# spaceandtimefdn/blitzar

Measured on NVIDIA H100. Metric: MSM throughput (scalar*point terms/sec), ristretto255, n=2^20 per GPU, higher is better.
Workload: dtype u32 limbs (integer modular arithmetic)

## Files before the change

### blitzar_b200/csrc/msm.cuh

```cuda
#pragma once
#include <algorithm>
#include <vector>

#include "batch_affine.cuh"
#include "curve.cuh"
#include "engine_api.cuh"
#include "lanefield.cuh"

namespace b200 {

struct ColumnDesc {
  const unsigned char* base;
  u64 row_stride;
  u32 bit_offset;
  u32 bit_width;
  u32 n;
  u32 is_signed;
  u32 first_window;
  u32 num_windows;
  u32 table_n;
  u32 gen_base;
};
B200_HD u32 bucket_windows(const ColumnDesc& col) { return col.table_n ? (col.num_windows ? 1u : 0u) : col.num_windows; }

B200_HD void load_scalar_bits(u32 v[8], bool& negative, const ColumnDesc& col, u64 i) {
  const unsigned char* row = col.base + i * col.row_stride;
#pragma unroll
  for (int k = 0; k < 8; ++k)
    v[k] = 0;
  const u32 width = col.bit_width;
  const unsigned char* p = row + (col.bit_offset >> 3);
  const u32 sh = col.bit_offset & 7u;
  if (sh == 0 && width == 256 && (((size_t)p) & 15u) == 0) {
    const uint4* q = (const uint4*)p;
    uint4 a = q[0], b = q[1];
    v[0] = a.x; v[1] = a.y; v[2] = a.z; v[3] = a.w;
    v[4] = b.x; v[5] = b.y; v[6] = b.z; v[7] = b.w;
  } else if (sh == 0 && (width & 31u) == 0 && (((size_t)p) & 3u) == 0) {
    const u32* q = (const u32*)p;
#pragma unroll
    for (int k = 0; k < 8; ++k)
      if ((u32)k < (width >> 5))
        v[k] = q[k];
  } else {
    const u32 nbytes = (sh + width + 7u) >> 3;
#pragma unroll
    for (int k = 0; k < 8; ++k) {
      u64 acc = 0;
#pragma unroll
      for (int b = 0; b < 5; ++b) {
        u32 idx = 4u * k + b;
        if (idx < nbytes)
          acc |= (u64)p[idx] << (8 * b);
      }
      v[k] = (u32)(acc >> sh);
    }
#pragma unroll
    for (int k = 0; k < 8; ++k) {
      int lo = 32 * k;
      if ((int)width <= lo)
        v[k] = 0;
      else if ((int)width < lo + 32)
        v[k] &= (1u << (width - lo)) - 1u;
    }
  }
  negative = false;
  if (col.is_signed) {
    u32 top = width - 1;
    bool neg = false;
#pragma unroll
    for (int k = 0; k < 8; ++k)
      if ((top >> 5) == (u32)k)
        neg = (v[k] >> (top & 31u)) & 1u;
    if (neg) {
      u64 c = 1;
#pragma unroll
      for (int k = 0; k < 8; ++k) {
        int lo = 32 * k;
        u32 m = 0;
        if ((int)width >= lo + 32)
          m = 0xffffffffu;
        else if ((int)width > lo)
          m = (1u << (width - lo)) - 1u;
        c += (u64)((~v[k]) & m);
        v[k] = (u32)c & m;
        c = (m == 0xffffffffu) ? (c >> 32) : 0;
      }
      negative = true;
    }
  }
}

constexpr u32 kAllWindows = 0xffffffffu;
template <class Fn>
B200_HD void for_each_digit(const u32 v[8], bool negative, const ColumnDesc& col, u32 c,
                            u32 nbuckets, Fn f, u32 only_window = kAllWindows) {
  const u32 half = nbuckets;
  const u32 mask = (1u << c) - 1u;
  u64 buf = 0;
  u32 nb = 0, w = 0, carry = 0;
  const u32 W = only_window == kAllWindows
                    ? col.num_windows
                    : (only_window < col.num_windows ? only_window + 1 : 0u);
  const auto step = [&] {
    u32 d = ((u32)buf & mask) + carry;
    buf >>= c;
    bool dneg = d > half;
    carry = dneg ? 1u : 0u;
    if (dneg)
      d = (1u << c) - d;
    if (d && (only_window == kAllWindows || w == only_window))
      f((col.first_window + (col.table_n ? 0u : w)) * nbuckets + (d - 1u), negative != dneg, w);
    ++w;
  };
#pragma unroll
  for (int k = 0; k < 8; ++k) {
    buf |= (u64)v[k] << nb;
    nb += 32;
    for (; nb >= c && w < W; nb -= c)
      step();
  }
  while (w < W)
    step();
}

B200_HD u32 column_of(const u64* col_start, u32 ncols, u64 tid) {
  u32 lo = 0, hi = ncols;
  while (hi - lo > 1) {
    const u32 mid = (lo + hi) >> 1;
    if (tid >= col_start[mid])
      lo = mid;
    else
      hi = mid;
  }
  return lo;
}
template <class Fn>
B200_HD void for_each_entry(const ColumnDesc* cols, const u64* col_start, u32 ncols, u32 c,
                            u32 nbuckets, u64 tid, Fn f, u32 only_window = kAllWindows) {
  const u32 j = column_of(col_start, ncols, tid);
  const ColumnDesc col = cols[j];
  if (only_window != kAllWindows && only_window >= col.num_windows)
    return;
  const u64 i = tid - col_start[j];
  u32 v[8];
  bool neg;
  load_scalar_bits(v, neg, col, i);
  const u32 ii = (u32)i + col.gen_base, tn = col.table_n;
  for_each_digit(v, neg, col, c, nbuckets, [&](u32 key, bool negate, u32 w) {
    f(key, make_entry(key, ii + w * tn, negate));
  }, only_window);
}

struct CountBody {
  static constexpr int kBlock = 256;
  const ColumnDesc* cols;
  const u64* col_start;
  u32 ncols, c, nbuckets;
  u32* counts;
  B200_HD void operator()(u64 tid) const {
    u32* cnt = counts;
    for_each_entry(cols, col_start, ncols, c, nbuckets, tid,
                   [cnt](u32 key, u64) { B200_ATOMIC_ADD(&cnt[key], 1u); });
  }
};

struct ScatterBody {
  static constexpr int kBlock = 256;
  const ColumnDesc* cols;
  const u64* col_start;
  u32 ncols, c, nbuckets;
  u32* cursor;
  u64* entries;
  u64 total_terms;
  B200_HD void operator()(u64 tid) const {
    u32 only = kAllWindows;
    if (total_terms) {
      only = (u32)(tid / total_terms);
      tid -= (u64)only * total_terms;
    }
    u32* cur = cursor;
    u64* en = entries;
    for_each_entry(cols, col_start, ncols, c, nbuckets, tid,
                   [cur, en](u32 key, u64 e) { en[B200_ATOMIC_ADD(&cur[key], 1u)] = e; }, only);
  }
};

constexpr u32 kScanChunk = 256, kScanChunkFirst = 64;
struct ScanUpBody {
  static constexpr int kBlock = 128;
  const u32* in;
  u64 n;
  u32* partial;
  u32 chunk;
  B200_HD void operator()(u64 t) const {
    u64 b = t * chunk, e = b + chunk < n ? b + chunk : n;
    u32 s = 0;
    for (u64 i = b; i < e; ++i)
      s += in[i];
    partial[t] = s;
  }
};
struct ScanTopBody {
  static constexpr int kBlock = 32;
  u32* data;
  u64 n;
  B200_HD void operator()(u64) const {
    u32 s = 0;
    for (u64 i = 0; i < n; ++i) {
      u32 v = data[i];
      data[i] = s;
      s += v;
    }
  }
};
struct ScanDownBody {
  static constexpr int kBlock = 128;
  u32* data;
  u64 n;
  const u32* partial_scanned;
  u32 chunk;
  B200_HD void operator()(u64 t) const {
    u64 b = t * chunk, e = b + chunk < n ? b + chunk : n;
    u32 s = partial_scanned[t];
    for (u64 i = b; i < e; ++i) {
      u32 v = data[i];
      data[i] = s;
      s += v;
    }
  }
};

inline void exclusive_scan(u32* data, u64 n, stream_t s, u32 chunk = kScanChunkFirst) {
  if (n <= kScanChunk) {
    launch(ScanTopBody{data, n}, 1, s);
    return;
  }
  u64 m = (n + chunk - 1) / chunk;
  u32* partial = (u32*)dev_alloc(m * sizeof(u32), s);
  launch(ScanUpBody{data, n, partial, chunk}, m, s);
  exclusive_scan(partial, m, s, kScanChunk);
  launch(ScanDownBody{data, n, partial, chunk}, m, s);
  dev_free(partial, s);
}

#if defined(__CUDACC__) && !defined(B200_EMULATE)
#define B200_BINNED_SORT 1
constexpr u32 kMicroBins = 16384, kBinCap = 8192, kBinSpan = 4096, kMaxBinShift = 12;
constexpr u64 kBinnedSortMinEntries = 1ull << 20;

template <int kBlock> __device__ u32 block_exclusive_scan(u32 v, u32* warp_sums, u32* total) {
  const u32 lane = threadIdx.x & 31u, warp = threadIdx.x >> 5;
  u32 x = v;
#pragma unroll
  for (int d = 1; d < 32; d <<= 1) {
    const u32 y = __shfl_up_sync(0xffffffffu, x, d);
    if (lane >= (u32)d)
      x += y;
  }
  if (lane == 31)
    warp_sums[warp] = x;
  __syncthreads();
  if (warp == 0) {
    u32 w = lane < kBlock / 32 ? warp_sums[lane] : 0u;
#pragma unroll
    for (int d = 1; d < 32; d <<= 1) {
      const u32 y = __shfl_up_sync(0xffffffffu, w, d);
      if (lane >= (u32)d)
        w += y;
    }
    if (lane < kBlock / 32)
      warp_sums[lane] = w;
  }
  __syncthreads();
  const u32 pre = (warp ? warp_sums[warp - 1] : 0u) + x - v;
  *total = warp_sums[kBlock / 32 - 1];
  __syncthreads();
  return pre;
}

struct MicroCountBody {
  static constexpr int kBlock = 512;
  const ColumnDesc* cols;
  const u64* col_start;
  u32 ncols, c, nbuckets;
  u64 total_terms;
  u32 tile, shift, nmicro;
  u32* micro_counts;
  __device__ void run(u32 b, unsigned char* smem) const {
    u32* h = (u32*)smem;
    for (u32 m = threadIdx.x; m < nmicro; m += kBlock)
      h[m] = 0;
    __syncthreads();
    const u64 lo = (u64)b * tile, hi = lo + tile < total_terms ? lo + tile : total_terms;
    const u32 sh = shift;
    for (u64 t = lo + threadIdx.x; t < hi; t += kBlock)
      for_each_entry(cols, col_start, ncols, c, nbuckets, t,
                     [h, sh](u32 key, u64) { atomicAdd(&h[key >> sh], 1u); });
    __syncthreads();
    for (u32 m = threadIdx.x; m < nmicro; m += kBlock)
      if (h[m])
        atomicAdd(&micro_counts[m], h[m]);
  }
};

struct PlanBinsBody {
  static constexpr int kBlock = 1024;
  const u32* micro_counts;
  u32 nmicro, span_micro;
  u64 nkeys;
  u32* bin_of;
  u32* bin_start;
  u32* bin_micro;
  u32* bin_cursor;
  u32* nbins_out;
  u32* counts;
  u32* d_m;
  __device__ bool starts_bin(const u32* st, u32 m) const {
    constexpr u32 H = kBinCap / 2;
    return m == 0 || m % span_micro == 0 || micro_counts[m] > H || micro_counts[m - 1] > H ||
           st[m] / H != st[m - 1] / H;
  }
  __device__ void run(u32, unsigned char* smem) const {
    __shared__ u32 ws[32];
    u32* st = (u32*)smem;
    const u32 per = (nmicro + kBlock - 1) / kBlock, m0 = min(threadIdx.x * per, nmicro),
              m1 = min(m0 + per, nmicro);
    u32 sum = 0;
    for (u32 m = m0; m < m1; ++m)
      sum += micro_counts[m];
    u32 total;
    u32 run = block_exclusive_scan<kBlock>(sum, ws, &total);
    for (u32 m = m0; m < m1; ++m) {
      st[m] = run;
      run += micro_counts[m];
    }
    __syncthreads();
    u32 nf = 0;
    for (u32 m = m0; m < m1; ++m)
      nf += starts_bin(st, m) ? 1u : 0u;
    u32 nbins;
    u32 id = block_exclusive_scan<kBlock>(nf, ws, &nbins);
    for (u32 m = m0; m < m1; ++m) {
      if (starts_bin(st, m)) {
        bin_start[id] = st[m];
        bin_micro[id] = m;
        bin_cursor[id] = st[m];
        ++id;
      }
      bin_of[m] = id - 1;
    }
    if (threadIdx.x == 0) {
      bin_start[nbins] = total;
      bin_micro[nbins] = nmicro;
      *nbins_out = nbins;
      counts[nkeys] = total;
      d_m[0] = total;
    }
  }
};

struct CoarseScatterBody {
  static constexpr int kBlock = 1024;
  const ColumnDesc* cols;
  const u64* col_start;
  u32 ncols, c, nbuckets;
  u64 total_terms;
  u32 tile, shift, nmicro;
  const u32* bin_of;
  const u32* nbins_ptr;
  u32* bin_cursor;
  u64* tmp;
  __device__ void run(u32 b, unsigned char* smem) const {
    __shared__ u32 ws[32];
    u32* h = (u32*)smem;
    u32* delta = h + nmicro;
    u64* stage = (u64*)(delta + nmicro + (nmicro & 1u));
    const u32 nbins = *nbins_ptr;
    for (u32 k = threadIdx.x; k < nbins; k += kBlock)
      h[k] = 0;
    __syncthreads();
    const u64 lo = (u64)b * tile, hi = lo + tile < total_terms ? lo + tile : total_terms;
    const u32 sh = shift;
    const u32* map = bin_of;
    for (u64 t = lo + threadIdx.x; t < hi; t += kBlock)
      for_each_entry(cols, col_start, ncols, c, nbuckets, t,
                     [h, sh, map](u32 key, u64) { atomicAdd(&h[__ldg(&map[key >> sh])], 1u); });
    __syncthreads();
    const u32 per = (nbins + kBlock - 1) / kBlock, k0 = min(threadIdx.x * per, nbins),
              k1 = min(k0 + per, nbins);
    u32 sum = 0;
    for (u32 k = k0; k < k1; ++k)
      sum += h[k];
    u32 size;
    u32 run = block_exclusive_scan<kBlock>(sum, ws, &size);
    for (u32 k = k0; k < k1; ++k) {
      const u32 n = h[k];
      if (n)
        delta[k] = atomicAdd(&bin_cursor[k], n) - run;
      h[k] = run;
      run += n;
    }
    __syncthreads();
    for (u64 t = lo + threadIdx.x; t < hi; t += kBlock)
      for_each_entry(cols, col_start, ncols, c, nbuckets, t, [h, sh, map, stage](u32 key, u64 e) {
        stage[atomicAdd(&h[__ldg(&map[key >> sh])], 1u)] = e;
      });
    __syncthreads();
    for (u32 i = threadIdx.x; i < size; i += kBlock) {
      const u64 e = stage[i];
      tmp[delta[__ldg(&map[entry_key(e) >> sh])] + i] = e;
    }
  }
};

struct BinSortBody {
  static constexpr int kBlock = 1024;
  static constexpr size_t kSmem = 2 * kBinCap * sizeof(u64) + kBinSpan * sizeof(u32);
  const u64* tmp;
  const u32* bin_start;
  const u32* bin_micro;
  const u32* nbins_ptr;
  u32 shift;
  u64 nkeys;
  u64* entries;
  u32* counts;
  __device__ void run(u32 b, unsigned char* smem) const {
    __shared__ u32 ws[32];
    if (b >= *nbins_ptr)
      return;
    u64* ent = (u64*)smem;
    u32* h = (u32*)(smem + 2 * kBinCap * sizeof(u64));
    const u32 lo = bin_start[b], size = bin_start[b + 1] - lo;
    const u64 klo = (u64)bin_micro[b] << shift, khi_m = (u64)bin_micro[b + 1] << shift;
    const u32 span = (u32)((khi_m < nkeys ? khi_m : nkeys) - klo);
    const bool local = size <= kBinCap;
    for (u32 k = threadIdx.x; k < span; k += kBlock)
      h[k] = 0;
    if (local) {
#pragma unroll 4
      for (u32 i = threadIdx.x; i < size; i += kBlock)
        ent[i] = tmp[(u64)lo + i];
    }
    __syncthreads();
    for (u32 i = threadIdx.x; i < size; i += kBlock) {
      const u64 e = local ? ent[i] : tmp[(u64)lo + i];
      atomicAdd(&h[entry_key(e) - (u32)klo], 1u);
    }
    __syncthreads();
    const u32 per = (span + kBlock - 1) / kBlock, k0 = min(threadIdx.x * per, span),
              k1 = min(k0 + per, span);
    u32 sum = 0;
    for (u32 k = k0; k < k1; ++k)
      sum += h[k];
    u32 total;
    u32 run = block_exclusive_scan<kBlock>(sum, ws, &total);
    for (u32 k = k0; k < k1; ++k) {
      const u32 n = h[k];
      h[k] = run;
      run += n;
      counts[klo + k] = lo + run;
    }
    __syncthreads();
    if (!local) {
      for (u32 i = threadIdx.x; i < size; i += kBlock) {
        const u64 e = tmp[(u64)lo + i];
        entries[(u64)lo + atomicAdd(&h[entry_key(e) - (u32)klo], 1u)] = e;
      }
      return;
    }
    u64* sorted = ent + kBinCap;
    for (u32 i = threadIdx.x; i < size; i += kBlock) {
      const u64 e = ent[i];
      sorted[atomicAdd(&h[entry_key(e) - (u32)klo], 1u)] = e;
    }
    __syncthreads();
    for (u32 i = threadIdx.x; i < size; i += kBlock)
      entries[(u64)lo + i] = sorted[i];
  }
};

inline u32 binned_sort_shift(u64 nkeys) {
  u32 shift = 0;
  while ((nkeys + (1ull << shift) - 1) >> shift > kMicroBins)
    ++shift;
  return shift;
}

inline void binned_sort(stream_t s, const ColumnDesc* d_cols, const u64* d_col_start, u32 ncols,
                        u32 c, u32 nbuckets, u64 total_terms, u64 max_entries, u32 max_windows,
                        u64 nkeys, u64* entries, u32* counts, u32* d_m) {
  const u32 shift = binned_sort_shift(nkeys);
  const u32 nmicro = (u32)((nkeys + (1ull << shift) - 1) >> shift);
  const u32 span_micro = std::max(1u, kBinSpan >> shift);
  u32* ws = (u32*)dev_alloc((5ull * nmicro + 3) * sizeof(u32), s);
  u32 *micro_counts = ws, *bin_of = ws + nmicro, *bin_cursor = ws + 2ull * nmicro,
      *bin_start = ws + 3ull * nmicro, *bin_micro = ws + 4ull * nmicro + 1,
      *nbins = ws + 5ull * nmicro + 2;
  u64* tmp = (u64*)dev_alloc(std::max<u64>(max_entries, 1) * sizeof(u64), s);
  dev_zero(micro_counts, nmicro * sizeof(u32), s);
  const u64 count_tile = 4096;
  launch_blocks(MicroCountBody{d_cols, d_col_start, ncols, c, nbuckets, total_terms,
                               (u32)count_tile, shift, nmicro, micro_counts},
                (total_terms + count_tile - 1) / count_tile, nmicro * sizeof(u32), s);
  launch_blocks(PlanBinsBody{micro_counts, nmicro, span_micro, nkeys, bin_of, bin_start, bin_micro,
                             bin_cursor, nbins, counts, d_m},
                1, nmicro * sizeof(u32), s);
  const size_t scatter_smem = 220 * 1024;
  const size_t bin_bytes = (2ull * nmicro + 2) * sizeof(u32);
  const u64 stage_entries = (scatter_smem - bin_bytes) / sizeof(u64);
  const u64 scatter_tile = std::max<u64>(1, stage_entries / max_windows);
  launch_blocks(CoarseScatterBody{d_cols, d_col_start, ncols, c, nbuckets, total_terms,
                                  (u32)scatter_tile, shift, nmicro, bin_of, nbins, bin_cursor, tmp},
                (total_terms + scatter_tile - 1) / scatter_tile, scatter_smem, s);
  launch_blocks(BinSortBody{tmp, bin_start, bin_micro, nbins, shift, nkeys, entries, counts}, nmicro,
                BinSortBody::kSmem, s);
  dev_free(tmp, s);
  dev_free(ws, s);
}
#endif

template <class C> struct FillIdentityBody {
  static constexpr int kBlock = 256;
  static constexpr u32 kChunks = sizeof(typename C::Point) / 16;
  static_assert(sizeof(typename C::Point) % 16 == 0, "points are made of 16-byte aligned fields");
  uint4* p;
  B200_HD void operator()(u64 t) const {
    const typename C::Point id = C::identity();
    const u32 k = (u32)(t % kChunks);
    uint4 v = ((const uint4*)&id)[0];
#pragma unroll
    for (u32 j = 1; j < kChunks; ++j)
      if (j == k)
        v = ((const uint4*)&id)[j];
    p[t] = v;
  }
};
template <class C> inline void fill_identity(stream_t s, typename C::Point* p, u64 n) {
  launch(FillIdentityBody<C>{(uint4*)p}, n * FillIdentityBody<C>::kChunks, s);
}

struct BucketOffsets {
  const u32* ends;
  const u32* starts;
  B200_HD u32 begin(u64 k) const { return starts ? starts[k] : (k ? ends[k - 1] : 0u); }
  B200_HD u32 end(u64 k) const { return ends[k]; }
};

template <class C> struct MergeBucketsBody {
  static constexpr int kBlock = 128;
  BucketOffsets offsets;
  const typename C::Point* scratch;
  typename C::Point* buckets;
  B200_HD void operator()(u64 k) const {
    if (offsets.begin(k) == offsets.end(k))
      return;
    typename C::Point b = buckets[k];
    C::add(b, b, scratch[k]);
    buckets[k] = b;
  }
};

template <class C, bool kGather, class X = SeqExec, bool kUniform = false, bool kUnitZ = false>
struct AccumulateBody {
  static constexpr int kBlock = 128;
  static constexpr int kMinBlocks = !kGather ? 1 : (C::F::N > 8 ? 2 : 3);
  typedef typename C::Point Point;
  typedef typename C::Gen Gen;
  const u32* keys;
  const u64* entries;
  const Gen* gens;
  const Point* pieces;
  const u32* m_ptr;
  u32 K;
  u32 final_level;
  Point* buckets;
  u32* out_keys;
  Point* out_pieces;
  u32* out_m_ptr;
  const u32* unit_veto;

  B200_HD void close_run(u64 t, u32 key, const Point& acc, bool writer, bool& first_seg) const {
    if (final_level || !first_seg) {
      if (writer)
        buckets[key] = acc;
    } else if (writer) {
      out_keys[2 * t] = key;
      out_pieces[2 * t] = acc;
    }
    first_seg = false;
  }
  template <bool kUnit> B200_HD Gen load_gen(u32 idx) const {
    if constexpr (kUnit)
      return C::load_unit_gen(gens + idx);
    else
      return gens[idx];
  }
  template <bool kUnit>
  B200_HD void gather_walk(u64 t, u64 b, u64 e, bool writer, u32& cur, Point& acc,
                           bool& first_seg) const {
    u64 ent = entries[b];
    Gen g = load_gen<kUnit>(entry_gen(ent));
    cur = entry_key(ent);
    for (u64 i = b; i < e; ++i) {
      u64 ent_n = ent;
      Gen g_n = g;
      if (i + 1 < e) {
        ent_n = entries[i + 1];
        g_n = load_gen<kUnit>(entry_gen(ent_n));
      }
      const u32 k = entry_key(ent);
      const bool negate = entry_negate(ent);
      if (kUniform) {
        if (i == b || k != cur) {
          if (i != b) {
            close_run(t, cur, acc, writer, first_seg);
            cur = k;
          }
          acc = C::identity();
        }
        C::template add_gen<X>(acc, acc, g, negate, kUnit);
      } else {
        const bool start = i == b || k != cur;
        if (k != cur) {
          close_run(t, cur, acc, writer, first_seg);
          cur = k;
        }
        if (start)
          C::gen_to_point(acc, g, negate);
        else
          C::template add_gen<X>(acc, acc, g, negate, kUnit);
      }
      ent = ent_n;
      g = g_n;
    }
  }
  B200_HD void operator()(u64 tid) const {
    const u64 t = tid / X::kLanes;
    const bool writer = (tid % X::kLanes) == 0;
    const u64 M = *m_ptr;
    const u64 T = (M + K - 1) / K;
    if (tid == 0 && out_m_ptr)
      *out_m_ptr = final_level ? 0u : (u32)(2 * T);
    u64 b = t * K;
    if (b >= M)
      return;
    u64 e = b + K < M ? b + K : M;
    u32 cur;
    Point acc;
    bool first_seg = true;
    if constexpr (kGather) {
      if (kUnitZ && unit_veto && *unit_veto)
        gather_walk<false>(t, b, e, writer, cur, acc, first_seg);
      else
        gather_walk<kUnitZ>(t, b, e, writer, cur, acc, first_seg);
    } else {
      cur = keys[b];
      acc = pieces[b];
      for (u64 i = b + 1; i < e; ++i) {
        const u32 k = keys[i];
        if (k == cur) {
          C::template add<X>(acc, acc, pieces[i]);
        } else {
          close_run(t, cur, acc, writer, first_seg);
          cur = k;
          acc = pieces[i];
        }
// ... 480 lines not shown
    if (kCommit)
      C::store_commit_abi(out + i * C::kAbiCommitBytes, pts[i]);
    else
      C::store_proj_abi(out + i * C::kAbiProjBytes, pts[i]);
  }
};
template <class C>
inline void launch_store_commit(stream_t s, const typename C::Point* pts, unsigned char* out,
                                u64 count, bool lane_tail) {
#ifdef B200_LANE_TAIL
  if constexpr (C::kCurveId == kRistretto255) {
    if (lane_tail && count && count <= 4096) {
      launch(StoreLaneBody{pts, out, count}, (count + 2) / 3 * 32, s);
      return;
    }
  }
#endif
  launch(StoreBody<C, true>{pts, out}, count, s);
}
template <class C> struct GenToProjBody {
  static constexpr int kBlock = 64;
  const typename C::Gen* gens;
  unsigned char* out;
  B200_HD void operator()(u64 i) const {
    typename C::Point p;
    C::gen_to_point(p, gens[i], false);
    C::store_proj_abi(out + i * C::kAbiProjBytes, p);
  }
};
template <class C> struct SumPartsBody {
  static constexpr int kBlock = 32;
  const typename C::Point* parts;
  u32 nparts, count;
  typename C::Point* out;
  B200_HD void operator()(u64 j) const {
    typename C::Point acc = parts[j];
    for (u32 r = 1; r < nparts; ++r)
      C::add(acc, acc, parts[(u64)r * count + j]);
    out[j] = acc;
  }
};

inline u32 choose_window_bits(u64 max_n, u32 max_width, u32 ncols, size_t point_bytes) {
  const double kMaxBucketBytes = 3.0e9;
  u32 best = 2;
  double best_cost = 1e300;
  for (u32 c = 2; c <= 16; ++c) {
    double W = (double)(max_width / c + 1);
    if (c > 8 && W * (double)(1u << (c - 1)) * (double)ncols * (double)point_bytes > kMaxBucketBytes)
      break;
    double cost = W * ((double)max_n + 2.5 * (double)(1u << (c - 1)));
    if (cost < best_cost) {
      best_cost = cost;
      best = c;
    }
  }
  return best;
}

struct MsmPlan {
  u32 c = 0, nbuckets = 0, ncols = 0, total_windows = 0;
  u64 nkeys = 0, max_n = 0, total_terms = 0, total_entries = 0;
  std::vector<ColumnDesc> cols;
};

inline MsmPlan msm_make_plan(std::vector<ColumnDesc> cols, const MsmOptions& opt,
                             size_t point_bytes) {
  MsmPlan p;
  p.ncols = (u32)cols.size();
  u32 max_width = 1;
  for (auto& col : cols) {
    p.max_n = std::max<u64>(p.max_n, col.n);
    p.total_terms += col.n;
    if (col.n)
      max_width = std::max(max_width, col.bit_width);
  }
  p.c = opt.window_bits ? opt.window_bits
                        : choose_window_bits(p.max_n, max_width, p.ncols, point_bytes);
  p.nbuckets = 1u << (p.c - 1);
  u64 max_entries = 0;
  for (auto& col : cols) {
    col.first_window = p.total_windows;
    col.num_windows = col.n ? col.bit_width / p.c + 1 : 0;
    p.total_windows += bucket_windows(col);
    max_entries += (u64)col.n * col.num_windows;
    if (col.table_n)
      B200_REQUIRE((u64)col.table_n * col.num_windows < (1ull << 31), "generator table too large");
    if (col.n)
      B200_REQUIRE((u64)col.gen_base + col.n + (u64)(col.num_windows - 1) * col.table_n < (1ull << 31),
                   "generator index of a column too large");
  }
  p.nkeys = (u64)p.total_windows * p.nbuckets;
  p.total_entries = max_entries;
  B200_REQUIRE(p.nkeys < (1ull << 32), "too many buckets for one pass");
  p.cols = std::move(cols);
  return p;
}

struct StagedRange {
  const ColumnDesc* d_cols = nullptr;
  const u64* d_col_start = nullptr;
  u64 total_terms = 0, max_entries = 0;
  u32 max_windows = 0;
  StagedRange(stream_t s, const MsmPlan& plan, u64 begin, u64 end) {
    const u32 ncols = plan.ncols;
    std::vector<ColumnDesc> cols(plan.cols);
    std::vector<u64> col_start(ncols + 1, 0);
    for (u32 j = 0; j < ncols; ++j) {
      u64 lo = std::min<u64>(begin, cols[j].n), hi = std::min<u64>(end, cols[j].n);
      cols[j].base += lo * cols[j].row_stride;
      cols[j].n = (u32)(hi - lo);
      col_start[j + 1] = col_start[j] + cols[j].n;
      max_entries += (u64)cols[j].n * cols[j].num_windows;
      max_windows = std::max(max_windows, cols[j].n ? cols[j].num_windows : 0u);
    }
    total_terms = col_start[ncols];
    if (total_terms == 0)
      return;
    B200_REQUIRE(max_entries < (1ull << 32) && end - begin < (1ull << 31),
                 "too many (term, window) entries for one sort pass");
    const size_t desc_bytes = ncols * sizeof(ColumnDesc), start_bytes = (ncols + 1) * sizeof(u64);
    std::vector<unsigned char> stage(desc_bytes + start_bytes);
    std::memcpy(stage.data(), cols.data(), desc_bytes);
    std::memcpy(stage.data() + desc_bytes, col_start.data(), start_bytes);
    d_cols = (const ColumnDesc*)stage_to_device(s, stage.data(), stage.size());
    d_col_start = (const u64*)((const unsigned char*)d_cols + desc_bytes);
  }
};

struct SortedLayout {
  u64* entries;
  u32* counts;
  u32* starts;
  u32* d_m;
  u64 slots_max;
  bool binned;
  BucketOffsets offsets() const { return {counts, starts}; }
};

inline SortedLayout sort_entries(stream_t s, const MsmPlan& plan, const StagedRange& r, u32 L,
                                 const MsmOptions& opt, u32* window_used) {
  const u32 ncols = plan.ncols, c = plan.c, nbuckets = plan.nbuckets;
  const u64 nkeys = plan.nkeys, max_entries = r.max_entries, total_terms = r.total_terms;
  SortedLayout out{};
  out.slots_max = L ? ((max_entries + nkeys * ((1ull << L) - 1) + (1ull << L) - 1) >> L) << L : max_entries;
  out.counts = (u32*)dev_alloc((nkeys + 1) * sizeof(u32), s);
  out.d_m = (u32*)dev_alloc(16 * sizeof(u32), s);
  out.entries = (u64*)dev_alloc(out.slots_max * sizeof(u64), s);
#ifdef B200_BINNED_SORT
  out.binned = L == 0 && opt.sort_path != 0 && binned_sort_shift(nkeys) <= kMaxBinShift &&
               (opt.sort_path == 2 || max_entries >= kBinnedSortMinEntries);
  if (out.binned)
    binned_sort(s, r.d_cols, r.d_col_start, ncols, c, nbuckets, total_terms, max_entries,
                r.max_windows, nkeys, out.entries, out.counts, out.d_m);
#endif
  if (!out.binned) {
    dev_zero(out.counts, (nkeys + 1) * sizeof(u32), s);
    launch(CountBody{r.d_cols, r.d_col_start, ncols, c, nbuckets, out.counts}, total_terms, s);
    if (L)
      launch(PadCountsBody{out.counts, (1u << L) - 1u}, nkeys, s);
    exclusive_scan(out.counts, nkeys + 1, s);
    copy_d2d(out.d_m, out.counts + nkeys, sizeof(u32), s);
    if (L) {
      out.starts = (u32*)dev_alloc((nkeys + 1) * sizeof(u32), s);
      copy_d2d(out.starts, out.counts, (nkeys + 1) * sizeof(u32), s);
    }
    const bool window_major = opt.scatter_window_major && r.max_windows > 1;
    launch(ScatterBody{r.d_cols, r.d_col_start, ncols, c, nbuckets, out.counts, out.entries,
                       window_major ? total_terms : 0},
           window_major ? total_terms * r.max_windows : total_terms, s);
  }
  if (L)
    launch(FillPadsBody{out.starts, out.counts, out.entries}, nkeys, s);
  launch(WindowUsedBody{out.offsets(), nbuckets, window_used}, plan.total_windows, s);
  return out;
}

inline unsigned sort_selftest(stream_t s, std::vector<ColumnDesc> cols, u32 c) {
  MsmOptions opt;
  opt.window_bits = c;
  const MsmPlan plan = msm_make_plan(std::move(cols), opt, 160);
  const StagedRange r(s, plan, 0, plan.max_n);
  if (r.total_terms == 0)
    return ~0u;
  const u64 nkeys = plan.nkeys, M = r.max_entries;
  DevBuf<u32> window_used(plan.total_windows, s);
  opt.sort_path = 0;
  const SortedLayout a = sort_entries(s, plan, r, 0, opt, window_used.p);
  opt.sort_path = 2;
  const SortedLayout b = sort_entries(s, plan, r, 0, opt, window_used.p);
  std::vector<u32> ca(nkeys + 1), cb(nkeys + 1), m(1);
  std::vector<u64> ea(M), eb(M);
  copy_d2h(ca.data(), a.counts, (nkeys + 1) * sizeof(u32), s);
  copy_d2h(cb.data(), b.counts, (nkeys + 1) * sizeof(u32), s);
  copy_d2h(m.data(), b.d_m, sizeof(u32), s);
  copy_d2h(ea.data(), a.entries, M * sizeof(u64), s);
  copy_d2h(eb.data(), b.entries, M * sizeof(u64), s);
  stream_sync(s);
  for (void* p : {(void*)a.entries, (void*)a.counts, (void*)a.d_m, (void*)b.entries, (void*)b.counts,
                  (void*)b.d_m, (void*)r.d_cols})
    dev_free(p, s);
  if (!b.binned)
    return ~0u;
  unsigned bad = m[0] == ca[nkeys] ? 0u : 1u;
  for (u64 k = 0; k < nkeys; ++k) {
    const u32 lo = k ? ca[k - 1] : 0u, hi = ca[k];
    if (cb[k] != hi || hi < lo || hi > M) {
      ++bad;
      continue;
    }
    std::sort(ea.begin() + lo, ea.begin() + hi);
    std::sort(eb.begin() + lo, eb.begin() + hi);
    if (!std::equal(ea.begin() + lo, ea.begin() + hi, eb.begin() + lo))
      ++bad;
  }
  return bad;
}

struct RangeHook {
  virtual void before_range(u64 begin, u64 end) = 0;
  virtual void before_accumulate() {}
  virtual ~RangeHook() {}
};

template <class C>
stream_t chunk_walk(stream_t s, stream_t tail, WalkInput<C> walk, u32* d_m, bool unit,
                    const u32* unit_veto, typename C::Point* target, const MsmOptions& opt,
                    std::vector<void*>& to_free) {
  typedef typename C::Point Point;
  u32 K = opt.chunk1 ? std::max(opt.chunk1, 4u) : (walk.m_max >= (1ull << 23) ? 64u : 32u);
  const u32 chunkn = std::max(opt.chunkn, 4u);
  const u32* lvl_keys = nullptr;
  const Point* lvl_pieces = nullptr;
  stream_t cs = s;
  for (int level = 0;; ++level) {
    const bool final_level = walk.m_max <= K;
    u64 T = (walk.m_max + K - 1) / K;
    u32* out_keys = final_level ? nullptr : (u32*)dev_alloc(2 * T * sizeof(u32), cs);
    Point* out_pieces = final_level ? nullptr : (Point*)dev_alloc(2 * T * sizeof(Point), cs);
    to_free.insert(to_free.end(), {out_keys, out_pieces});
    u32* out_m = d_m + 1 + (level % 8);
    const auto launch_level = [&](auto body, u64 threads, stream_t st) {
      body = {lvl_keys, walk.entries, walk.gens, lvl_pieces, walk.m_ptr, K, final_level, target,
              out_keys, out_pieces, out_m, unit_veto};
      launch(body, threads, st);
    };
    if (level == 0) {
      const bool uniform =
          opt.uniform_add == 2 ? C::kCurveId == kRistretto255 : opt.uniform_add != 0;
      constexpr bool kEd = C::kCurveId == kRistretto255;
      const bool unit_path = kEd && unit;
      if (uniform && unit_path)
        launch_level(AccumulateBody<C, true, SeqExec, true, kEd>{}, T, s);
      else if (uniform)
        launch_level(AccumulateBody<C, true, SeqExec, true>{}, T, s);
      else if (unit_path)
        launch_level(AccumulateBody<C, true, SeqExec, false, kEd>{}, T, s);
      else
        launch_level(AccumulateBody<C, true>{}, T, s);
      KernelTimer::get().end(s);
      if (tail != s)
        stream_follow(tail, s);
      cs = tail;
    } else if (T <= opt.quad_threshold) {
      launch_level(AccumulateBody<C, false, QuadExec>{}, T * QuadExec::kLanes, cs);
    } else {
      launch_level(AccumulateBody<C, false>{}, T, cs);
    }
    if (final_level)
      break;
    lvl_keys = out_keys;
    lvl_pieces = out_pieces;
    walk.m_ptr = out_m;
    walk.m_max = 2 * T;
    K = chunkn;
  }
  return cs;
}

template <class C>
void msm_accumulate_range(stream_t s, const MsmPlan& plan, const typename C::Gen* gens, u64 begin,
                          u64 end, bool add_into, typename C::Point* d_buckets,
                          u32* d_window_used, const MsmOptions& opt, stream_t tail,
                          RangeHook* hook = nullptr) {
  const StagedRange r(s, plan, begin, end);
  if (r.total_terms == 0)
    return;
  gens += begin;
  StageRange nvtx_sort("msm: digit count + scan + scatter");
  const u64 max_entries = r.max_entries, nkeys = plan.nkeys;
  u32 L = 0;
  if constexpr (C::kBatchAffine) {
    const double mean = (double)max_entries / (double)nkeys;
    if (opt.pair_levels >= 0)
      L = (u32)opt.pair_levels;
    else if (max_entries >= (1ull << 23))
      while (L < 6 && (double)(32u << L) <= mean)
        ++L;
    while (L > 0 && max_entries + nkeys * ((1ull << L) - 1) >= (1ull << 32) - (1ull << L))
      --L;
  }
  const SortedLayout sorted = sort_entries(s, plan, r, L, opt, d_window_used);
  B200_LOG(3, "range [%llu, %llu): %llu terms, %llu entries max, c=%u, %llu keys, pair levels %u",
           (unsigned long long)begin, (unsigned long long)end, (unsigned long long)r.total_terms,
           (unsigned long long)max_entries, plan.c, (unsigned long long)nkeys, L);
  WalkInput<C> walk{gens, sorted.entries, sorted.d_m, max_entries};
  std::vector<void*> to_free;
// ... 142 lines not shown
```

Baseline: 351.3 million.

## Restructure coarse scatter into per-window-group passes with cached digits and ranks

The coarse scatter kernel now splits work across blocks by term tile and by groups of three windows. Each block recodes scalar digits once into shared memory, ranks entries per bin with shared atomics, and scatters them through a per-window-set local bin map. This removes the second recode pass and the global bin_of lookups per entry, and shrinks shared histograms to one window set's bins. The tile count is sized to the SM count. The cost is more complex shared-memory layout and control flow, plus extra passes per window with a risk of lower occupancy or smaller tiles.

```diff
diff --git a/blitzar_b200/csrc/msm.cuh b/blitzar_b200/csrc/msm.cuh
--- a/blitzar_b200/csrc/msm.cuh
+++ b/blitzar_b200/csrc/msm.cuh
@@ -66,13 +66,12 @@
   }
   negative = false;
   if (col.is_signed) {
-    u32 top = width - 1;
-    bool neg = false;
+    const u32 top = width - 1;
+    u32 word = 0;
 #pragma unroll
     for (int k = 0; k < 8; ++k)
-      if ((top >> 5) == (u32)k)
-        neg = (v[k] >> (top & 31u)) & 1u;
-    if (neg) {
+      word |= v[k] & (0u - (u32)((top >> 5) == (u32)k));
+    if ((word >> (top & 31u)) & 1u) {
       u64 c = 1;
 #pragma unroll
       for (int k = 0; k < 8; ++k) {
@@ -93,15 +92,15 @@
 
 constexpr u32 kAllWindows = 0xffffffffu;
 template <class Fn>
-B200_HD void for_each_digit(const u32 v[8], bool negative, const ColumnDesc& col, u32 c,
-                            u32 nbuckets, Fn f, u32 only_window = kAllWindows) {
+B200_HD u32 for_each_digit(const u32 v[8], bool negative, const ColumnDesc& col, u32 c,
+                           u32 nbuckets, Fn f, u32 first = 0, u32 last = kAllWindows,
+                           u32 carry = 0) {
   const u32 half = nbuckets;
   const u32 mask = (1u << c) - 1u;
   u64 buf = 0;
-  u32 nb = 0, w = 0, carry = 0;
-  const u32 W = only_window == kAllWindows
-                    ? col.num_windows
-                    : (only_window < col.num_windows ? only_window + 1 : 0u);
+  u32 nb = 0, w = first;
+  const u32 W = last < col.num_windows ? last : col.num_windows;
+  const u32 skip = first * c;
   const auto step = [&] {
     u32 d = ((u32)buf & mask) + carry;
     buf >>= c;
@@ -109,19 +108,25 @@
     carry = dneg ? 1u : 0u;
     if (dneg)
       d = (1u << c) - d;
-    if (d && (only_window == kAllWindows || w == only_window))
+    if (d)
       f((col.first_window + (col.table_n ? 0u : w)) * nbuckets + (d - 1u), negative != dneg, w);
     ++w;
   };
 #pragma unroll
   for (int k = 0; k < 8; ++k) {
-    buf |= (u64)v[k] << nb;
-    nb += 32;
+    if (w >= W)
+      break;
+    if (32u * k + 32u <= skip)
+      continue;
+    const u32 s = skip > 32u * k ? skip - 32u * k : 0u;
+    buf |= (u64)(v[k] >> s) << nb;
+    nb += 32 - s;
     for (; nb >= c && w < W; nb -= c)
       step();
   }
   while (w < W)
     step();
+  return carry;
 }
 
 B200_HD u32 column_of(const u64* col_start, u32 ncols, u64 tid) {
@@ -135,21 +140,33 @@
   }
   return lo;
 }
+B200_HD u64 row_entry(const ColumnDesc& col, u64 i, u32 key, bool negate, u32 w) {
+  return make_entry(key, (u32)i + col.gen_base + w * col.table_n, negate);
+}
+constexpr u32 kWalkCarry = 0xffffffffu;
 template <class Fn>
-B200_HD void for_each_entry(const ColumnDesc* cols, const u64* col_start, u32 ncols, u32 c,
-                            u32 nbuckets, u64 tid, Fn f, u32 only_window = kAllWindows) {
+B200_HD u32 for_each_row_entry(const u32 v[8], bool neg, const ColumnDesc& col, u64 i, u32 c,
+                               u32 nbuckets, Fn f, u32 first = 0, u32 last = kAllWindows,
+                               u32 carry = 0) {
+  if (carry == kWalkCarry)
+    carry = for_each_digit(v, neg, col, c, nbuckets, [](u32, bool, u32) {}, 0, first);
+  return for_each_digit(v, neg, col, c, nbuckets, [&](u32 key, bool negate, u32 w) {
+    f(key, row_entry(col, i, key, negate, w), w);
+  }, first, last, carry);
+}
+template <class Fn>
+B200_HD u32 for_each_entry(const ColumnDesc* cols, const u64* col_start, u32 ncols, u32 c,
+                           u32 nbuckets, u64 tid, Fn f, u32 first = 0, u32 last = kAllWindows,
+                           u32 carry = 0) {
   const u32 j = column_of(col_start, ncols, tid);
   const ColumnDesc col = cols[j];
-  if (only_window != kAllWindows && only_window >= col.num_windows)
-    return;
+  if (first >= col.num_windows)
+    return 0;
   const u64 i = tid - col_start[j];
   u32 v[8];
   bool neg;
   load_scalar_bits(v, neg, col, i);
-  const u32 ii = (u32)i + col.gen_base, tn = col.table_n;
-  for_each_digit(v, neg, col, c, nbuckets, [&](u32 key, bool negate, u32 w) {
-    f(key, make_entry(key, ii + w * tn, negate));
-  }, only_window);
+  return for_each_row_entry(v, neg, col, i, c, nbuckets, f, first, last, carry);
 }
 
 struct CountBody {
@@ -161,7 +178,7 @@
   B200_HD void operator()(u64 tid) const {
     u32* cnt = counts;
     for_each_entry(cols, col_start, ncols, c, nbuckets, tid,
-                   [cnt](u32 key, u64) { B200_ATOMIC_ADD(&cnt[key], 1u); });
+                   [cnt](u32 key, u64, u32) { B200_ATOMIC_ADD(&cnt[key], 1u); });
   }
 };
 
@@ -174,15 +191,18 @@
   u64* entries;
   u64 total_terms;
   B200_HD void operator()(u64 tid) const {
-    u32 only = kAllWindows;
+    u32 first = 0, last = kAllWindows, carry = 0;
     if (total_terms) {
-      only = (u32)(tid / total_terms);
-      tid -= (u64)only * total_terms;
+      first = (u32)(tid / total_terms);
+      tid -= (u64)first * total_terms;
+      last = first + 1;
+      carry = kWalkCarry;
     }
     u32* cur = cursor;
     u64* en = entries;
     for_each_entry(cols, col_start, ncols, c, nbuckets, tid,
-                   [cur, en](u32 key, u64 e) { en[B200_ATOMIC_ADD(&cur[key], 1u)] = e; }, only);
+                   [cur, en](u32 key, u64 e, u32) { en[B200_ATOMIC_ADD(&cur[key], 1u)] = e; }, first,
+                   last, carry);
   }
 };
 
@@ -296,7 +316,7 @@
     const u32 sh = shift;
     for (u64 t = lo + threadIdx.x; t < hi; t += kBlock)
       for_each_entry(cols, col_start, ncols, c, nbuckets, t,
-                     [h, sh](u32 key, u64) { atomicAdd(&h[key >> sh], 1u); });
+                     [h, sh](u32 key, u64, u32) { atomicAdd(&h[key >> sh], 1u); });
     __syncthreads();
     for (u32 m = threadIdx.x; m < nmicro; m += kBlock)
       if (h[m])
@@ -362,54 +382,126 @@
 
 struct CoarseScatterBody {
   static constexpr int kBlock = 1024;
+  static constexpr u32 kGroupWindows = 3;
+  static constexpr u32 kNone = ~0u;
+  static constexpr u32 stage_bytes(u32 wpp) {
+    return kGroupWindows * sizeof(u32) + wpp * (sizeof(u64) + sizeof(uint16_t));
+  }
   const ColumnDesc* cols;
   const u64* col_start;
   u32 ncols, c, nbuckets;
   u64 total_terms;
-  u32 tile, shift, nmicro;
+  u32 tile, cap, groups, shift;
+  u32 set_micro, set_bins;
   const u32* bin_of;
-  const u32* nbins_ptr;
   u32* bin_cursor;
   u64* tmp;
-  __device__ void run(u32 b, unsigned char* smem) const {
+  __device__ void pass(u32 j, u32 w0, u32 w_end, u32 wlo, u32 whi, u32 a, u32 e, u32 m_lo, u32 nm,
+                       bool recode, bool map, unsigned char* smem) const {
     __shared__ u32 ws[32];
     u32* h = (u32*)smem;
-    u32* delta = h + nmicro;
-    u64* stage = (u64*)(delta + nmicro + (nmicro & 1u));
-    const u32 nbins = *nbins_ptr;
-    for (u32 k = threadIdx.x; k < nbins; k += kBlock)
+    u32* delta = h + set_bins;
+    uint16_t* lbin = (uint16_t*)(delta + set_bins);
+    u64* ordered = (u64*)(smem + 8 * set_bins + ((2 * set_micro + 7) & ~7u));
+    u32* digits = (u32*)(ordered + cap);
+    uint16_t* rank = (uint16_t*)(digits + kGroupWindows * tile);
+    const u32 n = e - a, row0 = (u32)col_start[j];
+    if (recode) {
+      const ColumnDesc col = cols[j];
+      for (u32 t = a + threadIdx.x; t < e; t += 2 * kBlock) {
+        const u32 i = t - a;
+        const bool two = t + kBlock < e;
+        u32 v[2][8];
+        bool neg[2];
+        load_scalar_bits(v[0], neg[0], col, t - row0);
+        if (two)
+          load_scalar_bits(v[1], neg[1], col, t + kBlock - row0);
+#pragma unroll
+        for (u32 r = 0; r < 2; ++r) {
+          if (r && !two)
+            break;
+          const u32 ir = i + r * kBlock;
+          for (u32 k = w0; k < w_end; ++k)
+            digits[(k - w0) * tile + ir] = kNone;
+          for_each_row_entry(v[r], neg[r], col, t + r * kBlock - row0, c, nbuckets,
+                             [&](u32 key, u64 ent, u32 wk) {
+                               digits[(wk - w0) * tile + ir] = key << 1 | (u32)entry_negate(ent);
+                             }, w0, w_end, kWalkCarry);
+        }
+      }
+    }
+    const u32 sh = shift, bin_lo = bin_of[m_lo], nb = bin_of[m_lo + nm - 1] + 1 - bin_lo;
+    for (u32 k = threadIdx.x; k < nb; k += kBlock)
       h[k] = 0;
+    for (u32 k = threadIdx.x; map && k < nm; k += kBlock)
+      lbin[k] = (uint16_t)(bin_of[m_lo + k] - bin_lo);
     __syncthreads();
-    const u64 lo = (u64)b * tile, hi = lo + tile < total_terms ? lo + tile : total_terms;
-    const u32 sh = shift;
-    const u32* map = bin_of;
-    for (u64 t = lo + threadIdx.x; t < hi; t += kBlock)
-      for_each_entry(cols, col_start, ncols, c, nbuckets, t,
-                     [h, sh, map](u32 key, u64) { atomicAdd(&h[__ldg(&map[key >> sh])], 1u); });
+    for (u32 w = wlo; w < whi; ++w) {
+      const u32* digit = digits + (w - w0) * tile;
+      uint16_t* rk = rank + (w - wlo) * n;
+      for (u32 i = threadIdx.x; i < n; i += kBlock) {
+        const u32 d = digit[i];
+        if (d != kNone)
+          rk[i] = (uint16_t)atomicAdd(&h[lbin[(d >> (sh + 1)) - m_lo]], 1u);
+      }
+    }
     __syncthreads();
-    const u32 per = (nbins + kBlock - 1) / kBlock, k0 = min(threadIdx.x * per, nbins),
-              k1 = min(k0 + per, nbins);
+    const u32 per = (nb + kBlock - 1) / kBlock, k0 = min(threadIdx.x * per, nb),
+              k1 = min(k0 + per, nb);
     u32 sum = 0;
     for (u32 k = k0; k < k1; ++k)
       sum += h[k];
     u32 size;
     u32 run = block_exclusive_scan<kBlock>(sum, ws, &size);
     for (u32 k = k0; k < k1; ++k) {
-      const u32 n = h[k];
-      if (n)
-        delta[k] = atomicAdd(&bin_cursor[k], n) - run;
+      const u32 cnt = h[k];
+      if (cnt)
+        delta[k] = atomicAdd(&bin_cursor[bin_lo + k], cnt) - run;
       h[k] = run;
-      run += n;
+      run += cnt;
     }
     __syncthreads();
-    for (u64 t = lo + threadIdx.x; t < hi; t += kBlock)
-      for_each_entry(cols, col_start, ncols, c, nbuckets, t, [h, sh, map, stage](u32 key, u64 e) {
-        stage[atomicAdd(&h[__ldg(&map[key >> sh])], 1u)] = e;
-      });
+    for (u32 w = wlo; w < whi; ++w) {
+      const u32* digit = digits + (w - w0) * tile;
+      const uint16_t* rk = rank + (w - wlo) * n;
+      for (u32 i = threadIdx.x; i < n; i += kBlock) {
+        const u32 d = digit[i];
+        if (d != kNone)
+          ordered[h[lbin[(d >> (sh + 1)) - m_lo]] + rk[i]] =
+              row_entry(cols[j], a + i - row0, d >> 1, d & 1u, w);
+      }
+    }
     __syncthreads();
     for (u32 i = threadIdx.x; i < size; i += kBlock) {
-      const u64 e = stage[i];
-      tmp[delta[__ldg(&map[entry_key(e) >> sh])] + i] = e;
+      const u64 ent = ordered[i];
+      tmp[delta[lbin[(entry_key(ent) >> sh) - m_lo]] + i] = ent;
+    }
+    __syncthreads();
+  }
+  __device__ void run(u32 b, unsigned char* smem) const {
+    const u32 w0 = b % groups * kGroupWindows;
+    const u64 lo = (u64)(b / groups) * tile, hi = lo + tile < total_terms ? lo + tile : total_terms;
+    u32 mapped = ~0u;
+    for (u32 j = column_of(col_start, ncols, lo); j < ncols && col_start[j] < hi; ++j) {
+      const ColumnDesc col = cols[j];
+      const u32 a = (u32)(col_start[j] > lo ? col_start[j] : lo);
+      const u32 e = (u32)(col_start[j + 1] < hi ? col_start[j + 1] : hi);
+      const u32 w_end = min(w0 + kGroupWindows, col.num_windows);
+      for (u32 w = w0; a < e && w < w_end; ++w) {
+        const u64 set = col.first_window + (col.table_n ? 0u : w);
+        const u32 m_lo = (u32)((set * nbuckets) >> shift);
+        const u32 nm = (u32)((((set + 1) * nbuckets - 1) >> shift) + 1 - m_lo);
+        if (col.table_n) {
+          const u32 len = cap / (w_end - w0);
+          for (u32 s0 = a; s0 < e; s0 += len) {
+            pass(j, w0, w_end, w0, w_end, s0, min(s0 + len, e), m_lo, nm, true, m_lo != mapped, smem);
+            mapped = m_lo;
+          }
+          break;
+        }
+        pass(j, w0, w_end, w, w + 1, a, e, m_lo, nm, w == w0, m_lo != mapped, smem);
+        mapped = m_lo;
+      }
     }
   }
 };
@@ -489,7 +581,7 @@
 
 inline void binned_sort(stream_t s, const ColumnDesc* d_cols, const u64* d_col_start, u32 ncols,
                         u32 c, u32 nbuckets, u64 total_terms, u64 max_entries, u32 max_windows,
-                        u64 nkeys, u64* entries, u32* counts, u32* d_m) {
+                        u64 nkeys, bool fixed_base, u64* entries, u32* counts, u32* d_m) {
   const u32 shift = binned_sort_shift(nkeys);
   const u32 nmicro = (u32)((nkeys + (1ull << shift) - 1) >> shift);
   const u32 span_micro = std::max(1u, kBinSpan >> shift);
@@ -506,13 +598,27 @@
   launch_blocks(PlanBinsBody{micro_counts, nmicro, span_micro, nkeys, bin_of, bin_start, bin_micro,
                              bin_cursor, nbins, counts, d_m},
                 1, nmicro * sizeof(u32), s);
+  const u32 set_micro =
+      std::min<u32>(nmicro, (u32)((nbuckets + (1ull << shift) - 1) >> shift) + 1);
+  const u64 plan_bins = 3 + nkeys / kBinSpan + 3 * max_entries / (kBinCap / 2);
+  const u32 set_bins = (u32)std::min<u64>(set_micro, plan_bins);
+  const u32 wpp = fixed_base ? CoarseScatterBody::kGroupWindows : 1u;
   const size_t scatter_smem = 220 * 1024;
-  const size_t bin_bytes = (2ull * nmicro + 2) * sizeof(u32);
-  const u64 stage_entries = (scatter_smem - bin_bytes) / sizeof(u64);
-  const u64 scatter_tile = std::max<u64>(1, stage_entries / max_windows);
+  const size_t bin_bytes = 8ull * set_bins + ((2ull * set_micro + 7) & ~7ull);
+  const u64 max_tile = (scatter_smem - bin_bytes) / CoarseScatterBody::stage_bytes(wpp);
+  constexpr u32 kGroup = CoarseScatterBody::kGroupWindows;
+  const u32 groups = (max_windows + kGroup - 1) / kGroup;
+  int dev = 0, sms = 0;
+  B200_CUDA(cudaGetDevice(&dev));
+  B200_CUDA(cudaDeviceGetAttribute(&sms, cudaDevAttrMultiProcessorCount, dev));
+  const u64 tiles = std::min<u64>(
+      std::max<u64>((total_terms + max_tile - 1) / max_tile, ((u64)sms + groups - 1) / groups),
+      std::max<u64>(total_terms, 1));
+  const u64 scatter_tile = (total_terms + tiles - 1) / tiles;
   launch_blocks(CoarseScatterBody{d_cols, d_col_start, ncols, c, nbuckets, total_terms,
-                                  (u32)scatter_tile, shift, nmicro, bin_of, nbins, bin_cursor, tmp},
-                (total_terms + scatter_tile - 1) / scatter_tile, scatter_smem, s);
+                                  (u32)scatter_tile, (u32)scatter_tile * wpp, groups, shift, set_micro,
+                                  set_bins, bin_of, bin_cursor, tmp},
+                tiles * groups, scatter_smem, s);
   launch_blocks(BinSortBody{tmp, bin_start, bin_micro, nbins, shift, nkeys, entries, counts}, nmicro,
                 BinSortBody::kSmem, s);
   dev_free(tmp, s);
@@ -1299,7 +1405,10 @@
                (opt.sort_path == 2 || max_entries >= kBinnedSortMinEntries);
   if (out.binned)
     binned_sort(s, r.d_cols, r.d_col_start, ncols, c, nbuckets, total_terms, max_entries,
-                r.max_windows, nkeys, out.entries, out.counts, out.d_m);
+                r.max_windows, nkeys,
+                std::all_of(plan.cols.begin(), plan.cols.end(),
+                            [](const ColumnDesc& col) { return col.table_n != 0; }),
+                out.entries, out.counts, out.d_m);
 #endif
   if (!out.binned) {
     dev_zero(out.counts, (nkeys + 1) * sizeof(u32), s);
```

Result: faster. 366.4 million, median of 6 (+4.3%).
